# aoschu/esn-ofdm-mimo

Measured on AMD Instinct MI355X. Metric: OFDM symbols/s through the ESN detector (4x8 TDL-B, N=128, N_res=512; train+predict+detect), higher is better.
Workload: dtype f16 operands / f32 accumulate

## Files before the change

### esn_ofdm_mimo_amd/csrc/esn_solve.hip

```cpp
#include <stdlib.h>
#include "esn_common.h"

namespace esn {

struct SolveParams {
    const double* E; const double* D;
    const float* E32;
    int n_groups, T, transient, cols, n_out;
    const double* t_scale; const double* t_shift;
    double* W_out; int* status;
    double* work; size_t work_stride;
    int m, n, wide;
    int skip;
    int part_ok;
};

__device__ __forceinline__ double wave_sum(double v) {
#pragma unroll
    for (int off = 32; off > 0; off >>= 1) v += __shfl_down(v, off);
    return __shfl(v, 0);
}

__global__ __launch_bounds__(1024) void readout_qr_kernel(SolveParams sp) {
    __shared__ double red[16];
    __shared__ double bc[4];
    const int g = blockIdx.x;
    const int tid = threadIdx.x, nth = blockDim.x;
    const int lane = tid & 63, wv = tid >> 6, nwv = nth >> 6;
    const int m = sp.m, n = sp.n, nrhs = sp.n_out;
    const int rows = sp.T - sp.transient, cols = sp.cols;
    double* M = sp.work + (size_t)g * sp.work_stride;
    const int ncol_tot = sp.wide ? n : n + nrhs;
    double* R = M + (size_t)ncol_tot * m;
    double* rdiag = R + (size_t)nrhs * m;
    double* beta = rdiag + n;
    const double* Eg = sp.E + ((size_t)g * sp.T + sp.transient) * cols;
    const double* Dg = sp.D + ((size_t)g * sp.T + sp.transient) * nrhs;

    if (sp.wide) {
        for (size_t i = tid; i < (size_t)n * m; i += nth) M[i] = Eg[i];
        for (int i = tid; i < nrhs * m; i += nth) {
            int o = i / m, j = i % m;
            double v = 0.0;
            if (j < n) {
                double sc = sp.t_scale ? sp.t_scale[(size_t)g * nrhs + o] : 1.0;
                double sh = sp.t_shift ? sp.t_shift[(size_t)g * nrhs + o] : 0.0;
                v = Dg[(size_t)j * nrhs + o] * sc + sh;
            }
            R[i] = v;
        }
    } else {
        for (size_t i = tid; i < (size_t)n * m; i += nth) {
            int c = (int)(i / m), rr = (int)(i % m);
            M[i] = Eg[(size_t)rr * cols + c];
        }
        for (int i = tid; i < nrhs * m; i += nth) {
            int o = i / m, rr = i % m;
            double sc = sp.t_scale ? sp.t_scale[(size_t)g * nrhs + o] : 1.0;
            double sh = sp.t_shift ? sp.t_shift[(size_t)g * nrhs + o] : 0.0;
            M[(size_t)(n + o) * m + rr] = Dg[(size_t)rr * nrhs + o] * sc + sh;
        }
    }
    __syncthreads();

    for (int j = 0; j < n; ++j) {
        double* cj = M + (size_t)j * m;
        double part = 0.0;
        for (int i = j + tid; i < m; i += nth) { double x = cj[i]; part = fma(x, x, part); }
        part = wave_sum(part);
        if (lane == 0) red[wv] = part;
        __syncthreads();
        if (tid == 0) {
            double sigma = 0.0;
            for (int w = 0; w < nwv; ++w) sigma += red[w];
            double x0 = cj[j];
            double nx = sqrt(sigma);
            double alpha = (x0 >= 0.0) ? -nx : nx;
            double v0 = x0 - alpha;
            double vtv = sigma - x0 * x0 + v0 * v0;
            double b = (vtv > 0.0) ? 2.0 / vtv : 0.0;
            cj[j] = v0;
            rdiag[j] = alpha;
            beta[j] = b;
            bc[0] = b;
        }
        __syncthreads();
        const double b = bc[0];
        if (b != 0.0) {
            for (int c = j + 1 + wv; c < ncol_tot; c += nwv) {
                double* cc = M + (size_t)c * m;
                double dot = 0.0;
                for (int i = j + lane; i < m; i += 64) dot = fma(cj[i], cc[i], dot);
                dot = wave_sum(dot) * b;
                for (int i = j + lane; i < m; i += 64) cc[i] = fma(-dot, cj[i], cc[i]);
            }
        }
        __syncthreads();
    }

    double rmax = 0.0;
    for (int j = tid; j < n; j += nth) rmax = fmax(rmax, fabs(rdiag[j]));
#pragma unroll
    for (int off = 32; off > 0; off >>= 1) rmax = fmax(rmax, __shfl_down(rmax, off));
    if (lane == 0) red[wv] = rmax;
    __syncthreads();
    if (tid == 0) {
        double r = 0.0;
        for (int w = 0; w < nwv; ++w) r = fmax(r, red[w]);
        bc[1] = r * 1e-13;
        int bad = 0;
        for (int j = 0; j < n; ++j) bad |= (fabs(rdiag[j]) <= r * 1e-13);
        sp.status[g] = bad ? 1 : 0;
    }
    __syncthreads();
    const double tol = bc[1];

    if (sp.wide) {
        for (int o = wv; o < nrhs; o += nwv) {
            double* z = R + (size_t)o * m;
            for (int j = 0; j < n; ++j) {
                const double* cj = M + (size_t)j * m;
                double acc = 0.0;
                for (int k = lane; k < j; k += 64) acc = fma(cj[k], z[k], acc);
                acc = wave_sum(acc);
                if (lane == 0) {
                    double d = rdiag[j];
                    z[j] = (fabs(d) > tol) ? (z[j] - acc) / d : 0.0;
                }
                __builtin_amdgcn_s_waitcnt(0);
                __builtin_amdgcn_wave_barrier();
            }
            for (int j = n - 1; j >= 0; --j) {
                const double* cj = M + (size_t)j * m;
                const double b = beta[j];
                if (b == 0.0) continue;
                double dot = 0.0;
                for (int i = j + lane; i < m; i += 64) dot = fma(cj[i], z[i], dot);
                dot = wave_sum(dot) * b;
                for (int i = j + lane; i < m; i += 64) z[i] = fma(-dot, cj[i], z[i]);
                __builtin_amdgcn_s_waitcnt(0);
                __builtin_amdgcn_wave_barrier();
            }
            double* wo = sp.W_out + ((size_t)g * nrhs + o) * cols;
            for (int i = lane; i < m; i += 64) wo[i] = z[i];
        }
    } else {
        for (int o = wv; o < nrhs; o += nwv) {
            double* c = M + (size_t)(n + o) * m;
            for (int j = n - 1; j >= 0; --j) {
                double acc = 0.0;
                for (int k = j + 1 + lane; k < n; k += 64) acc = fma(M[(size_t)k * m + j], c[k], acc);
                acc = wave_sum(acc);
                if (lane == 0) {
                    double d = rdiag[j];
                    c[j] = (fabs(d) > tol) ? (c[j] - acc) / d : 0.0;
                }
                __builtin_amdgcn_s_waitcnt(0);
                __builtin_amdgcn_wave_barrier();
            }
            double* wo = sp.W_out + ((size_t)g * nrhs + o) * cols;
            for (int i = lane; i < n; i += 64) wo[i] = c[i];
        }
    }
}

size_t solve_work_doubles(int rows, int cols, int n_out) {
    const bool wide = rows < cols;
    const size_t m = wide ? cols : rows, n = wide ? rows : cols;
    size_t d = (n + (wide ? 0 : n_out)) * m + (size_t)n_out * m + 2 * n;
    return (d + 1) & ~(size_t)1;
}

int launch_readout_solve(const double* E, const double* D, int n_groups, int T, int transient,
                         int cols, int n_out, const double* t_scale, const double* t_shift,
                         double* W_out, int* status, void* workspace, hipStream_t stream) {
    SolveParams sp;
    const int rows = T - transient;
    sp.E = E; sp.E32 = nullptr; sp.D = D; sp.n_groups = n_groups; sp.T = T; sp.transient = transient;
    sp.cols = cols; sp.n_out = n_out; sp.t_scale = t_scale; sp.t_shift = t_shift;
    sp.W_out = W_out; sp.status = status;
    sp.work = reinterpret_cast<double*>(workspace);
    sp.work_stride = solve_work_doubles(rows, cols, n_out);
    sp.wide = rows < cols;
    sp.m = sp.wide ? cols : rows;
    sp.n = sp.wide ? rows : cols;
    hipLaunchKernelGGL(readout_qr_kernel, dim3(n_groups), dim3(1024), 0, stream, sp);
    return (int)hipGetLastError();
}

}

namespace esn {

constexpr int CH_NP = 128;
constexpr int CH_LD = CH_NP + 1;
constexpr int CH_KC = 32;

__global__ __launch_bounds__(1024) void readout_chol_kernel(SolveParams sp) {
    extern __shared__ __attribute__((aligned(16))) char chol_smem[];
    double* Gs = reinterpret_cast<double*>(chol_smem);
    double* As = Gs;
    double* Bs = Gs + CH_NP * CH_LD;
    __shared__ int sh_bad;
    const int g = blockIdx.x, tid = threadIdx.x;
    const int lane = tid & 63, wv = tid >> 6;
    const int rows = sp.T - sp.transient, cols = sp.cols, nrhs = sp.n_out;
    const bool wide = rows < cols;
    const int n = wide ? rows : cols;
    const int m = wide ? cols : rows;
    const size_t a_off = ((size_t)g * sp.T + sp.transient) * cols;
    const double* A = sp.E ? sp.E + a_off : nullptr;
    const float* A32 = sp.E32 ? sp.E32 + a_off : nullptr;
    const double* Dg = sp.D + ((size_t)g * sp.T + sp.transient) * nrhs;
    constexpr int AS_LD = CH_NP + 4;

    const int wvu = __builtin_amdgcn_readfirstlane(wv);
    const int g_cnt = (wvu >> 2) == 0 ? 3 : 2;
    int g_ti[3], g_tj[3];
#pragma unroll
    for (int q = 0; q < 3; ++q) {
        const int m = wvu >> 2;
        const int idx = m == 0 ? q : 2 * m + 1 + (q < 2 ? q : 0);
        const int t = 4 * idx + (wvu & 3);
        int ti = 0;
        while ((ti + 1) * (ti + 2) / 2 <= t) ++ti;
        g_ti[q] = ti;
        g_tj[q] = t - ti * (ti + 1) / 2;
    }
    typedef double f64x4 __attribute__((ext_vector_type(4)));
    f64x4 acc[3];
#pragma unroll
    for (int q = 0; q < 3; ++q) acc[q] = f64x4{0.0, 0.0, 0.0, 0.0};
    const int fr_off = (lane >> 4) * (CH_NP + 4) + (lane & 15);
    double atb = 0.0;
    const int ao = tid / CH_NP, ai = tid % CH_NP;
    constexpr int EPT = CH_KC * CH_NP / 1024;
    double stgA[EPT], stgB[EPT];
    auto fetch = [&](double (&stg)[EPT], int k0) {
#pragma unroll
        for (int q = 0; q < EPT; ++q) {
            const int e = tid + 1024 * q;
            int kk, i;
            if (wide) { i = e / CH_KC; kk = e % CH_KC; } else { kk = e / CH_NP; i = e % CH_NP; }
            const int k = k0 + kk;
            const size_t ai_ = wide ? (size_t)i * cols + k : (size_t)k * cols + i;
            stg[q] = (i < n && k < m) ? (A32 ? (double)A32[ai_] : A[ai_]) : 0.0;
        }
    };
    auto commit = [&](const double (&stg)[EPT], double* dst) {
#pragma unroll
        for (int q = 0; q < EPT; ++q) {
            const int e = tid + 1024 * q;
            int kk, i;
            if (wide) { i = e / CH_KC; kk = e % CH_KC; } else { kk = e / CH_NP; i = e % CH_NP; }
            dst[kk * AS_LD + i] = stg[q];
        }
    };
    double* Abuf[2] = {As, As + CH_KC * AS_LD};
    const int m_run = (sp.skip & 1) ? CH_KC : m;
    auto chunk = [&](int k0, int cur, const double (&stg_next)[EPT], double (&stg_free)[EPT]) {
        if (k0 + 2 * CH_KC < m_run) fetch(stg_free, k0 + 2 * CH_KC);
        const double* Ac = Abuf[cur];
        const int kmax = (m - k0 < CH_KC) ? m - k0 : CH_KC;
#pragma unroll 2
        for (int k4 = 0; k4 < CH_KC; k4 += 4) {
            const double* slab = Ac + k4 * AS_LD + fr_off;
#pragma unroll
            for (int q = 0; q < 3; ++q)
                if (q < g_cnt)
                    acc[q] = __builtin_amdgcn_mfma_f64_16x16x4f64(slab[g_ti[q] * 16], slab[g_tj[q] * 16], acc[q], 0, 0, 0);
        }
        if (!wide && ao < nrhs) {
            const double sc = sp.t_scale ? sp.t_scale[(size_t)g * nrhs + ao] : 1.0;
            const double sh = sp.t_shift ? sp.t_shift[(size_t)g * nrhs + ao] : 0.0;
            for (int kk = 0; kk < kmax; ++kk)
                atb = fma(Ac[kk * AS_LD + ai], Dg[(size_t)(k0 + kk) * nrhs + ao] * sc + sh, atb);
        }
        if (k0 + CH_KC < m_run) commit(stg_next, Abuf[cur ^ 1]);
        __syncthreads();
    };
    fetch(stgA, 0);
    commit(stgA, Abuf[0]);
    if (CH_KC < m_run) fetch(stgA, CH_KC);
    __syncthreads();
    for (int k0 = 0; k0 < m_run; k0 += 2 * CH_KC) {
        chunk(k0, 0, stgA, stgB);
        if (k0 + CH_KC < m_run) chunk(k0 + CH_KC, 1, stgB, stgA);
    }
    __syncthreads();
#pragma unroll
    for (int q = 0; q < 3; ++q)
        if (q < g_cnt) {
#pragma unroll
            for (int i = 0; i < 4; ++i)
                Gs[(g_ti[q] * 16 + 4 * i + (lane >> 4)) * CH_LD + g_tj[q] * 16 + (lane & 15)] = acc[q][i];
        }
    if (tid == 0) sh_bad = 0;
    for (int e = tid; e < nrhs * CH_NP; e += 1024) {
        const int o = e / CH_NP, i = e % CH_NP;
        double v = 0.0;
        if (wide && i < n) {
            const double sc = sp.t_scale ? sp.t_scale[(size_t)g * nrhs + o] : 1.0;
            const double sh = sp.t_shift ? sp.t_shift[(size_t)g * nrhs + o] : 0.0;
            v = Dg[(size_t)i * nrhs + o] * sc + sh;
        }
        if (wide) Bs[e] = v;
    }
    __syncthreads();
    if (!wide && ao < nrhs) Bs[ao * CH_NP + ai] = (ai < n) ? atb : 0.0;
    double dmax = 0.0;
    if (tid < n) dmax = Gs[tid * CH_LD + tid];
#pragma unroll
    for (int off = 32; off > 0; off >>= 1) dmax = fmax(dmax, __shfl_down(dmax, off));
    __shared__ double sh_max[2];
    if (tid < 128 && lane == 0) sh_max[wv] = dmax;
    __syncthreads();
    const double piv_tol = fmax(sh_max[0], sh_max[1]) * 1e-14;

    __shared__ double sh_invd[CH_NP];
    __shared__ double sh_linv[16][17];
    auto bcast = [](double x, int src) -> double {
        const uint64_t u = __builtin_bit_cast(uint64_t, x);
        const uint32_t lo = __builtin_amdgcn_readlane((uint32_t)u, src);
        const uint32_t hi = __builtin_amdgcn_readlane((uint32_t)(u >> 32), src);
        return __builtin_bit_cast(double, ((uint64_t)hi << 32) | lo);
    };
    const int nblk = (sp.skip & 2) ? 1 : (n + 15) / 16;
    const int lr = lane & 15, lq = lane >> 4;
    for (int kb = 0; kb < nblk; ++kb) {
        const int j0 = 16 * kb;
        if (wv == 0) {
            const int r = lane & 15;
            double a[16], x[16];
#pragma unroll
            for (int c = 0; c < 16; ++c) a[c] = Gs[(j0 + r) * CH_LD + j0 + c];
            double my_invd = 1.0;
            unsigned rejected = 0;
#pragma unroll
            for (int j = 0; j < 16; ++j) {
                const double v = bcast(a[j], j);
                const bool live = j0 + j < n;
                const bool ok = live && v > piv_tol;
                if (live && !ok) rejected |= 1u << j;
                const double d = ok ? sqrt(v) : 1.0, inv_d = ok ? 1.0 / d : 0.0;
                if (r == j) my_invd = ok ? inv_d : 1.0;
                a[j] = (r == j) ? d : ((r > j) ? a[j] * inv_d : 0.0);
#pragma unroll
                for (int k = j + 1; k < 16; ++k) {
                    const double lkj = bcast(a[j], k);
                    if (r >= k) a[k] = fma(-a[j], lkj, a[k]);
                }
            }
            if (lane < 16) {
#pragma unroll
                for (int c = 0; c < 16; ++c) Gs[(j0 + r) * CH_LD + j0 + c] = a[c];
                sh_invd[j0 + r] = my_invd;
            }
            if (rejected && lane == 0) sh_bad = 1;
#pragma unroll
            for (int i = 0; i < 16; ++i) {
                double sacc = (i == r) ? 1.0 : 0.0;
#pragma unroll
                for (int k = 0; k < i; ++k) sacc = fma(-bcast(a[k], i), x[k], sacc);
                const double idi = bcast(my_invd, i);
                x[i] = (i >= r && !((rejected >> i) & 1u)) ? sacc * idi : 0.0;
            }
            if (lane < 16) {
#pragma unroll
                for (int i = 0; i < 16; ++i) sh_linv[i][r] = x[i];
            }
        }
        __syncthreads();
        const int ntile = (n + 15) / 16;
        {
            const int rt = kb + 1 + wv;
            if (rt < ntile) {
                f64x4 c = {0.0, 0.0, 0.0, 0.0};
#pragma unroll
                for (int k0 = 0; k0 < 16; k0 += 4)
                    c = __builtin_amdgcn_mfma_f64_16x16x4f64(Gs[(rt * 16 + lr) * CH_LD + j0 + k0 + lq],
                                                             sh_linv[lr][k0 + lq], c, 0, 0, 0);
#pragma unroll
                for (int i = 0; i < 4; ++i) Gs[(rt * 16 + 4 * i + lq) * CH_LD + j0 + lr] = c[i];
            }
        }
        __syncthreads();
        {
            const int mt = ntile - kb - 1, cnt = mt * (mt + 1) / 2;
            for (int t = wv; t < cnt; t += 16) {
                int di = 0;
                while ((di + 1) * (di + 2) / 2 <= t) ++di;
                const int ti = kb + 1 + di, tj = kb + 1 + t - di * (di + 1) / 2;
                f64x4 c;
#pragma unroll
                for (int i = 0; i < 4; ++i) c[i] = Gs[(ti * 16 + 4 * i + lq) * CH_LD + tj * 16 + lr];
#pragma unroll
                for (int k0 = 0; k0 < 16; k0 += 4)
                    c = __builtin_amdgcn_mfma_f64_16x16x4f64(-Gs[(ti * 16 + lr) * CH_LD + j0 + k0 + lq],
                                                             Gs[(tj * 16 + lr) * CH_LD + j0 + k0 + lq], c, 0, 0, 0);
#pragma unroll
                for (int i = 0; i < 4; ++i) Gs[(ti * 16 + 4 * i + lq) * CH_LD + tj * 16 + lr] = c[i];
            }
        }
        __syncthreads();
    }

    for (int o = wv; o < ((sp.skip & 4) ? 0 : nrhs); o += 16) {
        double* x = Bs + o * CH_NP;
        double b0 = x[lane], b1 = x[lane + 64];
        for (int j = 0; j < n; ++j) {
            const double own = (j < 64) ? b0 : b1;
            const double zj = __shfl(own, j & 63) * sh_invd[j];
            if (lane == (j & 63)) { if (j < 64) b0 = zj; else b1 = zj; }
            const double l0 = (lane > j) ? Gs[lane * CH_LD + j] : 0.0;
            const double l1 = (lane + 64 > j && lane + 64 < n) ? Gs[(lane + 64) * CH_LD + j] : 0.0;
            b0 = fma(-l0, zj, b0);
            b1 = fma(-l1, zj, b1);
        }
        for (int j = n - 1; j >= 0; --j) {
            const double own = (j < 64) ? b0 : b1;
            const double xj = __shfl(own, j & 63) * sh_invd[j];
            if (lane == (j & 63)) { if (j < 64) b0 = xj; else b1 = xj; }
            const double* Lj = Gs + j * CH_LD;
            const double l0 = (lane < j) ? Lj[lane] : 0.0;
            const double l1 = (lane + 64 < j) ? Lj[lane + 64] : 0.0;
            b0 = fma(-l0, xj, b0);
            b1 = fma(-l1, xj, b1);
        }
        x[lane] = b0; x[lane + 64] = b1;
    }
    __syncthreads();

    if (wide) {
        const int npair = cols / 2;
        if ((cols & 1) == 0 && 3 * npair <= 1024 && 3 * npair * 16 <= CH_NP * CH_LD && !(sp.skip & 8)) {
            double* part = Gs;
            const int third = tid / npair, pr = tid - third * npair;
            if (third < 3) {
                const int per = (n + 2) / 3;
                const int i0 = third * per, i1 = (i0 + per < n) ? i0 + per : n;
                double w0[8], w1[8];
#pragma unroll
                for (int o = 0; o < 8; ++o) { w0[o] = 0.0; w1[o] = 0.0; }
                const size_t ac = 2 * (size_t)pr;
#pragma unroll 8
                for (int i = i0; i < i1; ++i) {
                    double2 a;
                    if (A32) {
                        const float2 af = *reinterpret_cast<const float2*>(A32 + ac + (size_t)i * cols);
                        a = double2{(double)af.x, (double)af.y};
                    } else {
                        a = *reinterpret_cast<const double2*>(A + ac + (size_t)i * cols);
                    }
#pragma unroll
                    for (int o = 0; o < 8; ++o)
                        if (o < nrhs) {
                            const double al = Bs[o * CH_NP + i];
                            w0[o] = fma(a.x, al, w0[o]);
                            w1[o] = fma(a.y, al, w1[o]);
                        }
                }
#pragma unroll
                for (int o = 0; o < 8; ++o)
                    if (o < nrhs) {
                        part[(third * 8 + o) * cols + 2 * pr] = w0[o];
                        part[(third * 8 + o) * cols + 2 * pr + 1] = w1[o];
                    }
            }
            __syncthreads();
            for (int e = tid; e < nrhs * cols; e += 1024) {
                const int o = e / cols, c = e - o * cols;
                sp.W_out[((size_t)g * nrhs + o) * cols + c] =
                    (part[o * cols + c] + part[(8 + o) * cols + c]) + part[(16 + o) * cols + c];
            }
        } else {
            for (int c = tid; c < ((sp.skip & 8) ? 0 : cols); c += 1024) {
                double w[8];
#pragma unroll
                for (int o = 0; o < 8; ++o) w[o] = 0.0;
#pragma unroll 8
                for (int i = 0; i < n; ++i) {
                    const double a = A32 ? (double)A32[(size_t)i * cols + c] : A[(size_t)i * cols + c];
#pragma unroll
                    for (int o = 0; o < 8; ++o)
                        if (o < nrhs) w[o] = fma(a, Bs[o * CH_NP + i], w[o]);
                }
#pragma unroll
                for (int o = 0; o < 8; ++o)
                    if (o < nrhs) sp.W_out[((size_t)g * nrhs + o) * cols + c] = w[o];
            }
        }
    } else {
        for (int e = tid; e < nrhs * cols; e += 1024) {
            const int o = e / cols, c = e % cols;
            sp.W_out[((size_t)g * nrhs + o) * cols + c] = Bs[o * CH_NP + c];
        }
    }
    if (tid == 0) sp.status[g] = sh_bad;
}

int launch_readout_chol(const double* E, const float* E32, const double* D, int n_groups, int T, int transient,
                        int cols, int n_out, const double* t_scale, const double* t_shift,
                        double* W_out, int* status, hipStream_t stream) {
    SolveParams sp;
    sp.E32 = E32;
    const int rows = T - transient;
    const int n = rows < cols ? rows : cols;
    if (n > CH_NP || n_out > 8) return -1;
    sp.E = E; sp.D = D; sp.n_groups = n_groups; sp.T = T; sp.transient = transient;
    sp.cols = cols; sp.n_out = n_out; sp.t_scale = t_scale; sp.t_shift = t_shift;
    sp.W_out = W_out; sp.status = status; sp.work = nullptr; sp.work_stride = 0;
    sp.wide = rows < cols; sp.m = sp.wide ? cols : rows; sp.n = n;
    sp.skip = knobs().chol_skip;
    const size_t lds = sizeof(double) * ((size_t)CH_NP * CH_LD + (size_t)n_out * CH_NP);
    hipError_t e = hipFuncSetAttribute(reinterpret_cast<const void*>(readout_chol_kernel),
                                       hipFuncAttributeMaxDynamicSharedMemorySize, (int)lds);
    if (e != hipSuccess) return (int)e;
    hipLaunchKernelGGL(readout_chol_kernel, dim3(n_groups), dim3(1024), lds, stream, sp);
    return (int)hipGetLastError();
}

}

namespace esn {

constexpr int CB_NMAX = 512;
constexpr int CB_KC = 8;
constexpr int CB_PLD = 17;
constexpr int CB_NT = 512;
constexpr int CB_NW = CB_NT / 64;
constexpr int CB_EPT = CB_NMAX * CB_KC / CB_NT;
constexpr int CB_TPW = 16;

size_t chol_big_work_doubles(int n) {
    const size_t np = (size_t)round_up(n, 16);
    return np * np;
}

__global__ __launch_bounds__(CB_NT) void readout_chol_big_kernel(SolveParams sp) {
    extern __shared__ __attribute__((aligned(16))) char cb_smem[];
    typedef double f64x4 __attribute__((ext_vector_type(4)));
    __shared__ int sh_bad;
    __shared__ double sh_invd[CB_NMAX];
    __shared__ double sh_linv[16][17];
    __shared__ double sh_red[CB_NW];
    const int g = blockIdx.x, tid = threadIdx.x;
    const int lane = tid & 63, wv = tid >> 6;
    const int wvu = __builtin_amdgcn_readfirstlane(wv);
    const int rows = sp.T - sp.transient, cols = sp.cols, nrhs = sp.n_out;
    const bool wide = rows < cols;
    const int n = wide ? rows : cols;
    const int m = wide ? cols : rows;
    const int np = round_up(n, 16), ntile = np / 16;
    const int ld = np;
    double* Gw = sp.work + (size_t)g * sp.work_stride;
    const size_t a_off = ((size_t)g * sp.T + sp.transient) * cols;
    const double* A = sp.E ? sp.E + a_off : nullptr;
    const float* A32 = sp.E32 ? sp.E32 + a_off : nullptr;
    const double* Dg = sp.D + ((size_t)g * sp.T + sp.transient) * nrhs;
    const int lr = lane & 15, lq = lane >> 4;
    if (tid == 0) sh_bad = 0;

    {
        const int AS_LD = np + 4;
        double* Abuf[2] = {reinterpret_cast<double*>(cb_smem), reinterpret_cast<double*>(cb_smem) + (size_t)CB_KC * AS_LD};
        const int ept = (np * CB_KC + CB_NT - 1) / CB_NT;
        double stg[CB_EPT];
        auto fetch = [&](int k0) {
#pragma unroll
            for (int q = 0; q < CB_EPT; ++q) {
                const int e = tid + CB_NT * q;
                int kk, i;
                if (wide) { i = e / CB_KC; kk = e % CB_KC; } else { kk = e / np; i = e % np; }
                const int k = k0 + kk;
                const size_t ai_ = wide ? (size_t)i * cols + k : (size_t)k * cols + i;
                stg[q] = (q < ept && e < np * CB_KC && i < n && k < m) ? (A32 ? (double)A32[ai_] : A[ai_]) : 0.0;
            }
        };
        auto commit = [&](double* dst) {
#pragma unroll
            for (int q = 0; q < CB_EPT; ++q) {
                const int e = tid + CB_NT * q;
                if (q < ept && e < np * CB_KC) {
                    int kk, i;
                    if (wide) { i = e / CB_KC; kk = e % CB_KC; } else { kk = e / np; i = e % np; }
                    dst[kk * AS_LD + i] = stg[q];
                }
            }
        };
        const int fr_off = lq * AS_LD + lr;
        const int n_pass = (ntile + 3) / 4;
        for (int jb = 0; jb < n_pass; ++jb) {
            const int tj0 = 4 * jb, tj1 = (tj0 + 4 < ntile) ? tj0 + 4 : ntile;
            int cnt = 0;
            for (int tj = tj0; tj < tj1; ++tj) cnt += ntile - tj;
            int my_ti[CB_TPW], my_tj[CB_TPW];
#pragma unroll
            for (int q = 0; q < CB_TPW; ++q) {
                int t = wvu + CB_NW * q, tj = tj0;
                bool ok = t < cnt;
                while (ok && t >= ntile - tj) { t -= ntile - tj; ++tj; }
                my_tj[q] = ok ? tj : -1;
                my_ti[q] = ok ? tj + t : 0;
            }
            f64x4 acc[CB_TPW];
#pragma unroll
            for (int q = 0; q < CB_TPW; ++q) acc[q] = f64x4{0.0, 0.0, 0.0, 0.0};
            fetch(0);
            commit(Abuf[0]);
            __syncthreads();
            int cur = 0;
            for (int k0 = 0; k0 < m; k0 += CB_KC) {
                const bool more = k0 + CB_KC < m;
                if (more) fetch(k0 + CB_KC);
                const double* Ac = Abuf[cur];
#pragma unroll
                for (int k4 = 0; k4 < CB_KC; k4 += 4) {
                    const double* slab = Ac + k4 * AS_LD + fr_off;
#pragma unroll
                    for (int q = 0; q < CB_TPW; ++q)
                        if (my_tj[q] >= 0)
                            acc[q] = __builtin_amdgcn_mfma_f64_16x16x4f64(slab[my_ti[q] * 16], slab[my_tj[q] * 16], acc[q], 0, 0, 0);
                }
                if (more) commit(Abuf[cur ^ 1]);
                __syncthreads();
                cur ^= 1;
            }
#pragma unroll
            for (int q = 0; q < CB_TPW; ++q)
                if (my_tj[q] >= 0) {
#pragma unroll
                    for (int i = 0; i < 4; ++i)
                        Gw[(size_t)(my_tj[q] * 16 + lr) * ld + my_ti[q] * 16 + 4 * i + lq] = acc[q][i];
                }
            __syncthreads();
        }
        double* Bs = reinterpret_cast<double*>(cb_smem);
        __syncthreads();
        for (int e = tid; e < nrhs * np; e += CB_NT) {
            const int o = e / np, i = e % np;
            double v = 0.0;
            if (wide && i < n) {
                const double sc = sp.t_scale ? sp.t_scale[(size_t)g * nrhs + o] : 1.0;
                const double sh = sp.t_shift ? sp.t_shift[(size_t)g * nrhs + o] : 0.0;
                v = Dg[(size_t)i * nrhs + o] * sc + sh;
            }
            if (wide) Bs[e] = v;
        }
        if (!wide) {
            for (int e = tid; e < nrhs * np; e += CB_NT) {
                const int o = e / np, i = e % np;
                double acc_b = 0.0;
                if (i < n) {
                    const double sc = sp.t_scale ? sp.t_scale[(size_t)g * nrhs + o] : 1.0;
                    const double sh = sp.t_shift ? sp.t_shift[(size_t)g * nrhs + o] : 0.0;
#pragma unroll 8
                    for (int k = 0; k < m; ++k) {
                        const double a = A32 ? (double)A32[(size_t)k * cols + i] : A[(size_t)k * cols + i];
                        acc_b = fma(a, Dg[(size_t)k * nrhs + o] * sc + sh, acc_b);
                    }
                }
                Bs[e] = acc_b;
            }
        }
    }
    __threadfence_block();
    __syncthreads();
    double* Bs = reinterpret_cast<double*>(cb_smem);
    double* P = Bs + (size_t)8 * CB_NMAX;
    double dmax = 0.0;
    for (int i = tid; i < n; i += CB_NT) dmax = fmax(dmax, Gw[(size_t)i * ld + i]);
#pragma unroll
    for (int off = 32; off > 0; off >>= 1) dmax = fmax(dmax, __shfl_down(dmax, off));
    if (lane == 0) sh_red[wv] = dmax;
    __syncthreads();
    double piv_tol = 0.0;
    for (int w = 0; w < CB_NW; ++w) piv_tol = fmax(piv_tol, sh_red[w]);
    piv_tol *= 1e-14;

    auto bcast = [](double x, int src) -> double {
        const uint64_t u = __builtin_bit_cast(uint64_t, x);
        const uint32_t lo = __builtin_amdgcn_readlane((uint32_t)u, src);
        const uint32_t hi = __builtin_amdgcn_readlane((uint32_t)(u >> 32), src);
        return __builtin_bit_cast(double, ((uint64_t)hi << 32) | lo);
    };
    for (int j = 0; j < ntile; ++j) {
        const int j0 = 16 * j;
        for (int rt = j + wvu; rt < ntile; rt += CB_NW) {
            f64x4 c;
#pragma unroll
            for (int i = 0; i < 4; ++i) c[i] = Gw[(size_t)(j0 + lr) * ld + rt * 16 + 4 * i + lq];
            const double* la = Gw + (size_t)lq * ld + rt * 16 + lr;
            const double* lb = Gw + (size_t)lq * ld + j0 + lr;
#pragma unroll 4
            for (int k = 0; k < j0; k += 4)
                c = __builtin_amdgcn_mfma_f64_16x16x4f64(-la[(size_t)k * ld], lb[(size_t)k * ld], c, 0, 0, 0);
#pragma unroll
            for (int i = 0; i < 4; ++i) P[(rt * 16 + 4 * i + lq) * CB_PLD + lr] = c[i];
        }
        __syncthreads();
        if (wv == 0) {
            const int r = lane & 15;
            double a[16], x[16];
#pragma unroll
            for (int c = 0; c < 16; ++c) a[c] = P[(j0 + r) * CB_PLD + c];
            double my_invd = 1.0;
            unsigned rejected = 0;
#pragma unroll
            for (int jj = 0; jj < 16; ++jj) {
                const double v = bcast(a[jj], jj);
                const bool live = j0 + jj < n;
                const bool ok = live && v > piv_tol;
                if (live && !ok) rejected |= 1u << jj;
                const double d = ok ? sqrt(v) : 1.0, inv_d = ok ? 1.0 / d : 0.0;
                if (r == jj) my_invd = ok ? inv_d : 1.0;
                a[jj] = (r == jj) ? d : ((r > jj) ? a[jj] * inv_d : 0.0);
#pragma unroll
                for (int k = jj + 1; k < 16; ++k) {
                    const double lkj = bcast(a[jj], k);
                    if (r >= k) a[k] = fma(-a[jj], lkj, a[k]);
                }
            }
            if (lane < 16) {
#pragma unroll
                for (int c = 0; c < 16; ++c) P[(j0 + r) * CB_PLD + c] = a[c];
                sh_invd[j0 + r] = my_invd;
            }
            if (rejected && lane == 0) sh_bad = 1;
#pragma unroll
            for (int i = 0; i < 16; ++i) {
                double sacc = (i == r) ? 1.0 : 0.0;
#pragma unroll
                for (int k = 0; k < i; ++k) sacc = fma(-bcast(a[k], i), x[k], sacc);
                const double idi = bcast(my_invd, i);
                x[i] = (i >= r && !((rejected >> i) & 1u)) ? sacc * idi : 0.0;
            }
            if (lane < 16) {
#pragma unroll
                for (int i = 0; i < 16; ++i) sh_linv[i][r] = x[i];
            }
        }
        __syncthreads();
        for (int rt = j + 1 + wvu; rt < ntile; rt += CB_NW) {
            f64x4 c = {0.0, 0.0, 0.0, 0.0};
#pragma unroll
            for (int k0 = 0; k0 < 16; k0 += 4)
                c = __builtin_amdgcn_mfma_f64_16x16x4f64(P[(rt * 16 + lr) * CB_PLD + k0 + lq], sh_linv[lr][k0 + lq], c, 0, 0, 0);
            __builtin_amdgcn_wave_barrier();
#pragma unroll
            for (int i = 0; i < 4; ++i) P[(rt * 16 + 4 * i + lq) * CB_PLD + lr] = c[i];
        }
        __syncthreads();
        for (int e = tid; e < (np - j0) * 16; e += CB_NT) {
            const int c = e / (np - j0), rr = j0 + e % (np - j0);
            Gw[(size_t)(j0 + c) * ld + rr] = P[rr * CB_PLD + c];
        }
        __threadfence_block();
        __syncthreads();
    }

    if (wv < nrhs) {
        double* xb = Bs + (size_t)wv * np;
        constexpr int NS = CB_NMAX / 64;
        const int ns = (np + 63) / 64;
        double b[NS], l[NS], lnext[NS];
#pragma unroll
        for (int s2 = 0; s2 < NS; ++s2) b[s2] = (s2 < ns && lane + 64 * s2 < np) ? xb[lane + 64 * s2] : 0.0;
        auto load_col = [&](double (&dst)[NS], int jc) {
#pragma unroll
            for (int s2 = 0; s2 < NS; ++s2) {
                const int i = lane + 64 * s2;
                dst[s2] = (s2 < ns && jc >= 0 && jc < n && i < n) ? Gw[(size_t)jc * ld + i] : 0.0;
            }
        };
        auto pick = [&](const double (&v)[NS], int jc) -> double {
            double own = 0.0;
#pragma unroll
            for (int s2 = 0; s2 < NS; ++s2) own = ((jc >> 6) == s2) ? v[s2] : own;
            return __shfl(own, jc & 63);
        };
        load_col(l, 0);
        for (int jc = 0; jc < n; ++jc) {
            load_col(lnext, jc + 1);
            const double zj = pick(b, jc) * sh_invd[jc];
#pragma unroll
            for (int s2 = 0; s2 < NS; ++s2) {
                const int i = lane + 64 * s2;
                b[s2] = (i == jc) ? zj : ((i > jc) ? fma(-l[s2], zj, b[s2]) : b[s2]);
            }
#pragma unroll
            for (int s2 = 0; s2 < NS; ++s2) l[s2] = lnext[s2];
        }
        load_col(l, n - 1);
        for (int jc = n - 1; jc >= 0; --jc) {
            load_col(lnext, jc - 1);
            double part = 0.0;
#pragma unroll
            for (int s2 = 0; s2 < NS; ++s2) {
                const int i = lane + 64 * s2;
                part = (i > jc && i < n) ? fma(l[s2], b[s2], part) : part;
            }
            part = wave_sum(part);
            const double xj = (pick(b, jc) - part) * sh_invd[jc];
#pragma unroll
            for (int s2 = 0; s2 < NS; ++s2) b[s2] = (lane + 64 * s2 == jc) ? xj : b[s2];
#pragma unroll
            for (int s2 = 0; s2 < NS; ++s2) l[s2] = lnext[s2];
        }
#pragma unroll
        for (int s2 = 0; s2 < NS; ++s2)
            if (s2 < ns && lane + 64 * s2 < np) xb[lane + 64 * s2] = b[s2];
    }
    __syncthreads();

    if (wide) {
        double* part = P;
        if (sp.part_ok) {
            const int cpt = A32 ? 4 : 2, nunit = cols / cpt;
            int parts = CB_NT / nunit;
            if (parts > 3) parts = 3;
            const int pt = tid / nunit, un = tid - pt * nunit;
// ... 108 lines not shown
```

Baseline: 10.25 million.

## Restructure Cholesky readout kernel with packed tile storage and 512-thread blocks

Rewrites the small-n Cholesky readout solve to keep the Gram matrix as packed lower-triangular 16x16 tiles with an XOR swizzle, instead of a padded dense array. The block size drops from 1024 to 512 threads with a waves-per-EU hint so more blocks can be resident. The kernel is templated on element type and on wide/tall shape, and gains vectorised float4/double2 loads of E plus a column-vectorised W_out back-projection. The triangular solves use MFMA on the tiles, and fewer LDS bytes per block are meant to raise occupancy. In exchange each wave handles more tiles and the solve phases carry more synchronisation and complexity.

Result: faster. 10.88 million, median of 6 (+6.1%).

```diff
diff --git a/esn_ofdm_mimo_amd/csrc/esn_solve.hip b/esn_ofdm_mimo_amd/csrc/esn_solve.hip
--- a/esn_ofdm_mimo_amd/csrc/esn_solve.hip
+++ b/esn_ofdm_mimo_amd/csrc/esn_solve.hip
@@ -13,6 +13,7 @@
     int m, n, wide;
     int skip;
     int part_ok;
+    int vec;
 };
 
 __device__ __forceinline__ double wave_sum(double v) {
@@ -193,310 +194,407 @@
 namespace esn {
 
 constexpr int CH_NP = 128;
-constexpr int CH_LD = CH_NP + 1;
+constexpr int CH_NT = 512;
+constexpr int CH_NW = CH_NT / 64;
+constexpr int CH_TILES = 36;
 constexpr int CH_KC = 32;
-
-__global__ __launch_bounds__(1024) void readout_chol_kernel(SolveParams sp) {
+constexpr int CH_AS_LD = CH_NP + 16;
+constexpr int CH_RHS = 8;
+constexpr size_t CH_LDS = sizeof(double) * ((size_t)CH_TILES * 256 + (size_t)CH_NP * CH_RHS);
+static_assert(2 * CH_KC * CH_AS_LD <= CH_TILES * 256, "E staging aliases the Gram tiles");
+
+typedef double f64x4 __attribute__((ext_vector_type(4)));
+
+__device__ __forceinline__ int ch_tile(int ti, int tj) { return (ti * (ti + 1) / 2 + tj) * 256; }
+__device__ __forceinline__ int ch_el(int r, int c) { return r * 16 + (c ^ (r & ~1)); }
+
+__device__ __forceinline__ void ch_load4(const float* p, float (&v)[4]) {
+    const float4 x = *reinterpret_cast<const float4*>(p);
+    v[0] = x.x; v[1] = x.y; v[2] = x.z; v[3] = x.w;
+}
+__device__ __forceinline__ void ch_load4(const double* p, double (&v)[4]) {
+    const double2 x = *reinterpret_cast<const double2*>(p), y = *reinterpret_cast<const double2*>(p + 2);
+    v[0] = x.x; v[1] = x.y; v[2] = y.x; v[3] = y.y;
+}
+__device__ __forceinline__ const float* ch_src(const SolveParams& sp, float*) { return sp.E32; }
+__device__ __forceinline__ const double* ch_src(const SolveParams& sp, double*) { return sp.E; }
+
+__device__ __forceinline__ double ch_bcast(double x, int src) {
+    const uint64_t u = __builtin_bit_cast(uint64_t, x);
+    const uint32_t lo = __builtin_amdgcn_readlane((uint32_t)u, src);
+    const uint32_t hi = __builtin_amdgcn_readlane((uint32_t)(u >> 32), src);
+    return __builtin_bit_cast(double, ((uint64_t)hi << 32) | lo);
+}
+
+__device__ __forceinline__ int ch_factor_diag(double* D, int j0, int n, double piv_tol, int lane) {
+    const int r = lane & 15;
+    double a[16], x[16];
+#pragma unroll
+    for (int c = 0; c < 16; ++c) a[c] = D[ch_el(r, c)];
+    double my_invd = 1.0;
+    unsigned rejected = 0, dropped = 0;
+#pragma unroll
+    for (int j = 0; j < 16; ++j) {
+        const double v = ch_bcast(a[j], j);
+        const bool live = j0 + j < n;
+        const bool ok = live && v > piv_tol;
+        if (live && !ok) rejected |= 1u << j;
+        if (!ok) dropped |= 1u << j;
+        const double d = ok ? sqrt(v) : 1.0, inv_d = ok ? 1.0 / d : 0.0;
+        if (r == j) my_invd = ok ? inv_d : 1.0;
+        a[j] = (r == j) ? d : ((r > j) ? a[j] * inv_d : 0.0);
+#pragma unroll
+        for (int k = j + 1; k < 16; ++k) {
+            const double lkj = ch_bcast(a[j], k);
+            if (r >= k) a[k] = fma(-a[j], lkj, a[k]);
+        }
+    }
+#pragma unroll
+    for (int i = 0; i < 16; ++i) {
+        double sacc = (i == r) ? 1.0 : 0.0;
+#pragma unroll
+        for (int k = 0; k < i; ++k) sacc = fma(-ch_bcast(a[k], i), x[k], sacc);
+        const double idi = ch_bcast(my_invd, i);
+        x[i] = (i >= r && !((dropped >> i) & 1u)) ? sacc * idi : 0.0;
+    }
+    if (lane < 16) {
+#pragma unroll
+        for (int i = 0; i < 16; ++i) D[ch_el(i, r)] = x[i];
+    }
+    return rejected ? 1 : 0;
+}
+
+template <typename TE, bool wide>
+__global__ __launch_bounds__(CH_NT) __attribute__((amdgpu_waves_per_eu(4))) void readout_chol_kernel(SolveParams sp) {
     extern __shared__ __attribute__((aligned(16))) char chol_smem[];
     double* Gs = reinterpret_cast<double*>(chol_smem);
     double* As = Gs;
-    double* Bs = Gs + CH_NP * CH_LD;
-    __shared__ int sh_bad;
+    double* Bs = Gs + CH_TILES * 256;
     const int g = blockIdx.x, tid = threadIdx.x;
-    const int lane = tid & 63, wv = tid >> 6;
+    const int lane = tid & 63, wv = __builtin_amdgcn_readfirstlane(tid >> 6);
+    const int lr = lane & 15, lq = lane >> 4;
     const int rows = sp.T - sp.transient, cols = sp.cols, nrhs = sp.n_out;
-    const bool wide = rows < cols;
     const int n = wide ? rows : cols;
     const int m = wide ? cols : rows;
-    const size_t a_off = ((size_t)g * sp.T + sp.transient) * cols;
-    const double* A = sp.E ? sp.E + a_off : nullptr;
-    const float* A32 = sp.E32 ? sp.E32 + a_off : nullptr;
+    const int ntile = (n + 15) / 16;
+    const TE* A = ch_src(sp, (TE*)nullptr) + ((size_t)g * sp.T + sp.transient) * cols;
     const double* Dg = sp.D + ((size_t)g * sp.T + sp.transient) * nrhs;
-    constexpr int AS_LD = CH_NP + 4;
-
-    const int wvu = __builtin_amdgcn_readfirstlane(wv);
-    const int g_cnt = (wvu >> 2) == 0 ? 3 : 2;
-    int g_ti[3], g_tj[3];
-#pragma unroll
-    for (int q = 0; q < 3; ++q) {
-        const int m = wvu >> 2;
-        const int idx = m == 0 ? q : 2 * m + 1 + (q < 2 ? q : 0);
-        const int t = 4 * idx + (wvu & 3);
+
+    int g_ti[5], g_tj[5];
+    const int g_cnt = wv < 4 ? 5 : 4;
+#pragma unroll
+    for (int q = 0; q < 5; ++q) {
+        const int t = wv + CH_NW * q < CH_TILES ? wv + CH_NW * q : 0;
         int ti = 0;
         while ((ti + 1) * (ti + 2) / 2 <= t) ++ti;
         g_ti[q] = ti;
         g_tj[q] = t - ti * (ti + 1) / 2;
     }
-    typedef double f64x4 __attribute__((ext_vector_type(4)));
-    f64x4 acc[3];
-#pragma unroll
-    for (int q = 0; q < 3; ++q) acc[q] = f64x4{0.0, 0.0, 0.0, 0.0};
-    const int fr_off = (lane >> 4) * (CH_NP + 4) + (lane & 15);
-    double atb = 0.0;
-    const int ao = tid / CH_NP, ai = tid % CH_NP;
-    constexpr int EPT = CH_KC * CH_NP / 1024;
-    double stgA[EPT], stgB[EPT];
-    auto fetch = [&](double (&stg)[EPT], int k0) {
-#pragma unroll
-        for (int q = 0; q < EPT; ++q) {
-            const int e = tid + 1024 * q;
-            int kk, i;
-            if (wide) { i = e / CH_KC; kk = e % CH_KC; } else { kk = e / CH_NP; i = e % CH_NP; }
+    f64x4 acc[5];
+#pragma unroll
+    for (int q = 0; q < 5; ++q) acc[q] = f64x4{0.0, 0.0, 0.0, 0.0};
+    double atb[2] = {0.0, 0.0};
+    auto run_of = [&](int p, int& i, int& kk) {
+        const int e = tid + CH_NT * p;
+        if (wide) { i = (e & 15) + 16 * ((e >> 7) & 7); kk = 4 * ((e >> 4) & 7); }
+        else      { kk = e >> 5; i = 4 * (e & 31); }
+    };
+    TE stg[2][4];
+    auto fetch = [&](int k0) {
+#pragma unroll
+        for (int p = 0; p < 2; ++p) {
+            int i, kk;
+            run_of(p, i, kk);
             const int k = k0 + kk;
-            const size_t ai_ = wide ? (size_t)i * cols + k : (size_t)k * cols + i;
-            stg[q] = (i < n && k < m) ? (A32 ? (double)A32[ai_] : A[ai_]) : 0.0;
+            int nv = wide ? (i < n ? m - k : 0) : (k < m ? n - i : 0);
+            nv = nv < 0 ? 0 : (nv > 4 ? 4 : nv);
+            const TE* src = A + (wide ? (size_t)i * cols + k : (size_t)k * cols + i);
+            if (nv == 4 && sp.vec) {
+                ch_load4(src, stg[p]);
+            } else {
+#pragma unroll
+                for (int j = 0; j < 4; ++j) stg[p][j] = j < nv ? src[j] : (TE)0;
+            }
         }
     };
-    auto commit = [&](const double (&stg)[EPT], double* dst) {
-#pragma unroll
-        for (int q = 0; q < EPT; ++q) {
-            const int e = tid + 1024 * q;
-            int kk, i;
-            if (wide) { i = e / CH_KC; kk = e % CH_KC; } else { kk = e / CH_NP; i = e % CH_NP; }
-            dst[kk * AS_LD + i] = stg[q];
+    auto commit = [&](double* dst) {
+#pragma unroll
+        for (int p = 0; p < 2; ++p) {
+            int i, kk;
+            run_of(p, i, kk);
+#pragma unroll
+            for (int j = 0; j < 4; ++j) {
+                if (wide) dst[(kk + j) * CH_AS_LD + i] = (double)stg[p][j];
+                else      dst[kk * CH_AS_LD + i + j] = (double)stg[p][j];
+            }
         }
     };
-    double* Abuf[2] = {As, As + CH_KC * AS_LD};
+    double* Abuf[2] = {As, As + CH_KC * CH_AS_LD};
     const int m_run = (sp.skip & 1) ? CH_KC : m;
-    auto chunk = [&](int k0, int cur, const double (&stg_next)[EPT], double (&stg_free)[EPT]) {
-        if (k0 + 2 * CH_KC < m_run) fetch(stg_free, k0 + 2 * CH_KC);
+    for (int k0 = 0, cur = 0; k0 < m_run; k0 += CH_KC, cur ^= 1) {
+        if (k0 == 0) {
+            fetch(0);
+            commit(Abuf[0]);
+            __syncthreads();
+        }
+        if (k0 + CH_KC < m_run) fetch(k0 + CH_KC);
         const double* Ac = Abuf[cur];
         const int kmax = (m - k0 < CH_KC) ? m - k0 : CH_KC;
-#pragma unroll 2
-        for (int k4 = 0; k4 < CH_KC; k4 += 4) {
-            const double* slab = Ac + k4 * AS_LD + fr_off;
-#pragma unroll
-            for (int q = 0; q < 3; ++q)
+        const double* slab0 = Ac + lq * CH_AS_LD + lr;
+        for (int k4 = 0; k4 < kmax; k4 += 4) {
+            const double* slab = slab0 + k4 * CH_AS_LD;
+#pragma unroll
+            for (int q = 0; q < 5; ++q)
                 if (q < g_cnt)
                     acc[q] = __builtin_amdgcn_mfma_f64_16x16x4f64(slab[g_ti[q] * 16], slab[g_tj[q] * 16], acc[q], 0, 0, 0);
         }
-        if (!wide && ao < nrhs) {
-            const double sc = sp.t_scale ? sp.t_scale[(size_t)g * nrhs + ao] : 1.0;
-            const double sh = sp.t_shift ? sp.t_shift[(size_t)g * nrhs + ao] : 0.0;
-            for (int kk = 0; kk < kmax; ++kk)
-                atb = fma(Ac[kk * AS_LD + ai], Dg[(size_t)(k0 + kk) * nrhs + ao] * sc + sh, atb);
-        }
-        if (k0 + CH_KC < m_run) commit(stg_next, Abuf[cur ^ 1]);
-        __syncthreads();
-    };
-    fetch(stgA, 0);
-    commit(stgA, Abuf[0]);
-    if (CH_KC < m_run) fetch(stgA, CH_KC);
+        if constexpr (!wide) {
+#pragma unroll
+            for (int p = 0; p < 2; ++p) {
+                const int e = tid + CH_NT * p, o = e / CH_NP, i = e % CH_NP;
+                if (o < nrhs) {
+                    const double sc = sp.t_scale ? sp.t_scale[(size_t)g * nrhs + o] : 1.0;
+                    const double sh = sp.t_shift ? sp.t_shift[(size_t)g * nrhs + o] : 0.0;
+                    for (int kk = 0; kk < kmax; ++kk)
+                        atb[p] = fma(Ac[kk * CH_AS_LD + i], Dg[(size_t)(k0 + kk) * nrhs + o] * sc + sh, atb[p]);
+                }
+            }
+        }
+        if (k0 + CH_KC < m_run) commit(Abuf[cur ^ 1]);
+        __syncthreads();
+    }
+
+#pragma unroll
+    for (int q = 0; q < 5; ++q)
+        if (q < g_cnt) {
+            double* T = Gs + ch_tile(g_ti[q], g_tj[q]);
+#pragma unroll
+            for (int i = 0; i < 4; ++i) T[ch_el(4 * i + lq, lr)] = acc[q][i];
+        }
+#pragma unroll
+    for (int p = 0; p < 2; ++p) {
+        const int e = tid + CH_NT * p;
+        if (wide) {
+            const int i = e / CH_RHS, o = e % CH_RHS;
+            double v = 0.0;
+            if (i < n && o < nrhs) {
+                const double sc = sp.t_scale ? sp.t_scale[(size_t)g * nrhs + o] : 1.0;
+                const double sh = sp.t_shift ? sp.t_shift[(size_t)g * nrhs + o] : 0.0;
+                v = Dg[(size_t)i * nrhs + o] * sc + sh;
+            }
+            Bs[e] = v;
+        } else {
+            const int o = e / CH_NP, i = e % CH_NP;
+            Bs[i * CH_RHS + o] = (o < nrhs && i < n) ? atb[p] : 0.0;
+        }
+    }
     __syncthreads();
-    for (int k0 = 0; k0 < m_run; k0 += 2 * CH_KC) {
-        chunk(k0, 0, stgA, stgB);
-        if (k0 + CH_KC < m_run) chunk(k0 + CH_KC, 1, stgB, stgA);
-    }
-    __syncthreads();
-#pragma unroll
-    for (int q = 0; q < 3; ++q)
-        if (q < g_cnt) {
-#pragma unroll
-            for (int i = 0; i < 4; ++i)
-                Gs[(g_ti[q] * 16 + 4 * i + (lane >> 4)) * CH_LD + g_tj[q] * 16 + (lane & 15)] = acc[q][i];
-        }
-    if (tid == 0) sh_bad = 0;
-    for (int e = tid; e < nrhs * CH_NP; e += 1024) {
-        const int o = e / CH_NP, i = e % CH_NP;
-        double v = 0.0;
-        if (wide && i < n) {
-            const double sc = sp.t_scale ? sp.t_scale[(size_t)g * nrhs + o] : 1.0;
-            const double sh = sp.t_shift ? sp.t_shift[(size_t)g * nrhs + o] : 0.0;
-            v = Dg[(size_t)i * nrhs + o] * sc + sh;
-        }
-        if (wide) Bs[e] = v;
-    }
-    __syncthreads();
-    if (!wide && ao < nrhs) Bs[ao * CH_NP + ai] = (ai < n) ? atb : 0.0;
-    double dmax = 0.0;
-    if (tid < n) dmax = Gs[tid * CH_LD + tid];
-#pragma unroll
-    for (int off = 32; off > 0; off >>= 1) dmax = fmax(dmax, __shfl_down(dmax, off));
-    __shared__ double sh_max[2];
-    if (tid < 128 && lane == 0) sh_max[wv] = dmax;
-    __syncthreads();
-    const double piv_tol = fmax(sh_max[0], sh_max[1]) * 1e-14;
-
-    __shared__ double sh_invd[CH_NP];
-    __shared__ double sh_linv[16][17];
-    auto bcast = [](double x, int src) -> double {
-        const uint64_t u = __builtin_bit_cast(uint64_t, x);
-        const uint32_t lo = __builtin_amdgcn_readlane((uint32_t)u, src);
-        const uint32_t hi = __builtin_amdgcn_readlane((uint32_t)(u >> 32), src);
-        return __builtin_bit_cast(double, ((uint64_t)hi << 32) | lo);
-    };
-    const int nblk = (sp.skip & 2) ? 1 : (n + 15) / 16;
-    const int lr = lane & 15, lq = lane >> 4;
-    for (int kb = 0; kb < nblk; ++kb) {
-        const int j0 = 16 * kb;
-        if (wv == 0) {
-            const int r = lane & 15;
-            double a[16], x[16];
-#pragma unroll
-            for (int c = 0; c < 16; ++c) a[c] = Gs[(j0 + r) * CH_LD + j0 + c];
-            double my_invd = 1.0;
-            unsigned rejected = 0;
-#pragma unroll
-            for (int j = 0; j < 16; ++j) {
-                const double v = bcast(a[j], j);
-                const bool live = j0 + j < n;
-                const bool ok = live && v > piv_tol;
-                if (live && !ok) rejected |= 1u << j;
-                const double d = ok ? sqrt(v) : 1.0, inv_d = ok ? 1.0 / d : 0.0;
-                if (r == j) my_invd = ok ? inv_d : 1.0;
-                a[j] = (r == j) ? d : ((r > j) ? a[j] * inv_d : 0.0);
-#pragma unroll
-                for (int k = j + 1; k < 16; ++k) {
-                    const double lkj = bcast(a[j], k);
-                    if (r >= k) a[k] = fma(-a[j], lkj, a[k]);
-                }
-            }
-            if (lane < 16) {
-#pragma unroll
-                for (int c = 0; c < 16; ++c) Gs[(j0 + r) * CH_LD + j0 + c] = a[c];
-                sh_invd[j0 + r] = my_invd;
-            }
-            if (rejected && lane == 0) sh_bad = 1;
-#pragma unroll
-            for (int i = 0; i < 16; ++i) {
-                double sacc = (i == r) ? 1.0 : 0.0;
-#pragma unroll
-                for (int k = 0; k < i; ++k) sacc = fma(-bcast(a[k], i), x[k], sacc);
-                const double idi = bcast(my_invd, i);
-                x[i] = (i >= r && !((rejected >> i) & 1u)) ? sacc * idi : 0.0;
-            }
-            if (lane < 16) {
-#pragma unroll
-                for (int i = 0; i < 16; ++i) sh_linv[i][r] = x[i];
-            }
-        }
-        __syncthreads();
-        const int ntile = (n + 15) / 16;
-        {
+
+    int bad = 0;
+    const int nblk = (sp.skip & 2) ? 1 : ntile;
+    double piv_tol = 0.0;
+    if (wv == 0) {
+        double dmax = 0.0;
+        for (int i = lane; i < n; i += 64) dmax = fmax(dmax, Gs[ch_tile(i >> 4, i >> 4) + ch_el(i & 15, i & 15)]);
+#pragma unroll
+        for (int off = 32; off > 0; off >>= 1) dmax = fmax(dmax, __shfl_xor(dmax, off));
+        piv_tol = dmax * 1e-14;
+    }
+    for (int kb = -1; kb < nblk; ++kb) {
+        if (kb >= 0) {
             const int rt = kb + 1 + wv;
             if (rt < ntile) {
+                const double* Li = Gs + ch_tile(kb, kb);
+
+                double* T = Gs + ch_tile(rt, kb);
                 f64x4 c = {0.0, 0.0, 0.0, 0.0};
 #pragma unroll
                 for (int k0 = 0; k0 < 16; k0 += 4)
-                    c = __builtin_amdgcn_mfma_f64_16x16x4f64(Gs[(rt * 16 + lr) * CH_LD + j0 + k0 + lq],
-                                                             sh_linv[lr][k0 + lq], c, 0, 0, 0);
-#pragma unroll
-                for (int i = 0; i < 4; ++i) Gs[(rt * 16 + 4 * i + lq) * CH_LD + j0 + lr] = c[i];
-            }
-        }
-        __syncthreads();
-        {
+                    c = __builtin_amdgcn_mfma_f64_16x16x4f64(T[ch_el(lr, k0 + lq)], Li[ch_el(lr, k0 + lq)], c, 0, 0, 0);
+#pragma unroll
+                for (int i = 0; i < 4; ++i) T[ch_el(4 * i + lq, lr)] = c[i];
+            }
+        }
+        if (kb >= 0) {
+            __syncthreads();
             const int mt = ntile - kb - 1, cnt = mt * (mt + 1) / 2;
-            for (int t = wv; t < cnt; t += 16) {
+            for (int t = wv; t < cnt; t += (wv == 0 ? cnt : CH_NW - 1)) {
                 int di = 0;
                 while ((di + 1) * (di + 2) / 2 <= t) ++di;
                 const int ti = kb + 1 + di, tj = kb + 1 + t - di * (di + 1) / 2;
+                double* C = Gs + ch_tile(ti, tj);
+                const double* La = Gs + ch_tile(ti, kb);
+                const double* Lb = Gs + ch_tile(tj, kb);
                 f64x4 c;
 #pragma unroll
-                for (int i = 0; i < 4; ++i) c[i] = Gs[(ti * 16 + 4 * i + lq) * CH_LD + tj * 16 + lr];
+                for (int i = 0; i < 4; ++i) c[i] = C[ch_el(4 * i + lq, lr)];
 #pragma unroll
                 for (int k0 = 0; k0 < 16; k0 += 4)
-                    c = __builtin_amdgcn_mfma_f64_16x16x4f64(-Gs[(ti * 16 + lr) * CH_LD + j0 + k0 + lq],
-                                                             Gs[(tj * 16 + lr) * CH_LD + j0 + k0 + lq], c, 0, 0, 0);
-#pragma unroll
-                for (int i = 0; i < 4; ++i) Gs[(ti * 16 + 4 * i + lq) * CH_LD + tj * 16 + lr] = c[i];
-            }
-        }
-        __syncthreads();
-    }
-
-    for (int o = wv; o < ((sp.skip & 4) ? 0 : nrhs); o += 16) {
-        double* x = Bs + o * CH_NP;
-        double b0 = x[lane], b1 = x[lane + 64];
-        for (int j = 0; j < n; ++j) {
-            const double own = (j < 64) ? b0 : b1;
-            const double zj = __shfl(own, j & 63) * sh_invd[j];
-            if (lane == (j & 63)) { if (j < 64) b0 = zj; else b1 = zj; }
-            const double l0 = (lane > j) ? Gs[lane * CH_LD + j] : 0.0;
-            const double l1 = (lane + 64 > j && lane + 64 < n) ? Gs[(lane + 64) * CH_LD + j] : 0.0;
-            b0 = fma(-l0, zj, b0);
-            b1 = fma(-l1, zj, b1);
-        }
-        for (int j = n - 1; j >= 0; --j) {
-            const double own = (j < 64) ? b0 : b1;
-            const double xj = __shfl(own, j & 63) * sh_invd[j];
-            if (lane == (j & 63)) { if (j < 64) b0 = xj; else b1 = xj; }
-            const double* Lj = Gs + j * CH_LD;
-            const double l0 = (lane < j) ? Lj[lane] : 0.0;
-            const double l1 = (lane + 64 < j) ? Lj[lane + 64] : 0.0;
-            b0 = fma(-l0, xj, b0);
-            b1 = fma(-l1, xj, b1);
-        }
-        x[lane] = b0; x[lane + 64] = b1;
-    }
-    __syncthreads();
-
-    if (wide) {
-        const int npair = cols / 2;
-        if ((cols & 1) == 0 && 3 * npair <= 1024 && 3 * npair * 16 <= CH_NP * CH_LD && !(sp.skip & 8)) {
+                    c = __builtin_amdgcn_mfma_f64_16x16x4f64(-La[ch_el(lr, k0 + lq)], Lb[ch_el(lr, k0 + lq)], c, 0, 0, 0);
+#pragma unroll
+                for (int i = 0; i < 4; ++i) C[ch_el(4 * i + lq, lr)] = c[i];
+            }
+        }
+        if (wv == 0 && kb + 1 < nblk) bad |= ch_factor_diag(Gs + ch_tile(kb + 1, kb + 1), 16 * (kb + 1), n, piv_tol, lane);
+        __syncthreads();
+    }
+
+    if (!(sp.skip & 4)) {
+        const bool bl = lr < CH_RHS;
+        f64x4 keep = {0.0, 0.0, 0.0, 0.0};
+        int keep_t = -1;
+        auto rhs_tile = [&](int I) -> f64x4 {
+            f64x4 v;
+#pragma unroll
+            for (int i = 0; i < 4; ++i) v[i] = bl ? Bs[(16 * I + 4 * i + lq) * CH_RHS + lr] : 0.0;
+            return v;
+        };
+        auto put_tile = [&](int I, const f64x4& v) {
+            if (bl) {
+#pragma unroll
+                for (int i = 0; i < 4; ++i) Bs[(16 * I + 4 * i + lq) * CH_RHS + lr] = v[i];
+            }
+        };
+        auto flush = [&]() {
+            if (wv == CH_NW - 1 && keep_t >= 0) put_tile(keep_t, keep);
+            keep_t = -1;
+        };
+        for (int I = 0; I < ntile; ++I) {
+            flush();
+            const int J = I + 1 + wv;
+            const bool upd = J < ntile;
+            if (upd || wv == CH_NW - 1) {
+                const double* Li = Gs + ch_tile(I, I);
+                const f64x4 b = rhs_tile(I);
+                f64x4 z = {0.0, 0.0, 0.0, 0.0};
+#pragma unroll
+                for (int s = 0; s < 4; ++s)
+                    z = __builtin_amdgcn_mfma_f64_16x16x4f64(Li[ch_el(lr, 4 * s + lq)], b[s], z, 0, 0, 0);
+                if (upd) {
+                    const double* L = Gs + ch_tile(J, I);
+                    f64x4 c = rhs_tile(J);
+#pragma unroll
+                    for (int s = 0; s < 4; ++s)
+                        c = __builtin_amdgcn_mfma_f64_16x16x4f64(-L[ch_el(lr, 4 * s + lq)], z[s], c, 0, 0, 0);
+                    put_tile(J, c);
+                } else {
+                    keep = z;
+                    keep_t = I;
+                }
+            }
+            __syncthreads();
+        }
+        flush();
+        __syncthreads();
+        for (int I = ntile - 1; I >= 0; --I) {
+            flush();
+            const int J = wv;
+            const bool upd = J < I;
+            if (upd || wv == CH_NW - 1) {
+                const double* Li = Gs + ch_tile(I, I);
+                const f64x4 zi = rhs_tile(I);
+                f64x4 x = {0.0, 0.0, 0.0, 0.0};
+#pragma unroll
+                for (int s = 0; s < 4; ++s)
+                    x = __builtin_amdgcn_mfma_f64_16x16x4f64(Li[ch_el(4 * s + lq, lr)], zi[s], x, 0, 0, 0);
+                if (upd) {
+                    const double* L = Gs + ch_tile(I, J);
+                    f64x4 c = rhs_tile(J);
+#pragma unroll
+                    for (int s = 0; s < 4; ++s)
+                        c = __builtin_amdgcn_mfma_f64_16x16x4f64(-L[ch_el(4 * s + lq, lr)], x[s], c, 0, 0, 0);
+                    put_tile(J, c);
+                } else {
+                    keep = x;
+                    keep_t = I;
+                }
+            }
+            __syncthreads();
+        }
+        flush();
+        __syncthreads();
+    }
+
+    if constexpr (wide) {
+        constexpr int CPT = 16 / sizeof(TE);
+        const int nunit = cols / CPT;
+        int parts = nunit > 0 ? CH_NT / nunit : 0;
+        parts = parts > 3 ? 3 : parts;
+        if (sp.vec && cols % CPT == 0 && parts > 0 && (parts - 1) * CH_RHS * cols <= CH_TILES * 256 && !(sp.skip & 8)) {
             double* part = Gs;
-            const int third = tid / npair, pr = tid - third * npair;
-            if (third < 3) {
-                const int per = (n + 2) / 3;
-                const int i0 = third * per, i1 = (i0 + per < n) ? i0 + per : n;
-                double w0[8], w1[8];
-#pragma unroll
-                for (int o = 0; o < 8; ++o) { w0[o] = 0.0; w1[o] = 0.0; }
-                const size_t ac = 2 * (size_t)pr;
-#pragma unroll 8
+            const int pt = tid / nunit, un = tid - pt * nunit;
+            double w[CPT][CH_RHS];
+#pragma unroll
+            for (int c = 0; c < CPT; ++c)
+#pragma unroll
+                for (int o = 0; o < CH_RHS; ++o) w[c][o] = 0.0;
+            if (pt < parts) {
+                const int per = (n + parts - 1) / parts;
+                const int i0 = pt * per, i1 = (i0 + per < n) ? i0 + per : n;
+                const TE* ac = A + (size_t)CPT * un;
+#pragma unroll 4
                 for (int i = i0; i < i1; ++i) {
-                    double2 a;
-                    if (A32) {
-                        const float2 af = *reinterpret_cast<const float2*>(A32 + ac + (size_t)i * cols);
-                        a = double2{(double)af.x, (double)af.y};
+                    TE a[CPT];
+                    if constexpr (CPT == 4) {
+                        ch_load4(ac + (size_t)i * cols, a);
                     } else {
-                        a = *reinterpret_cast<const double2*>(A + ac + (size_t)i * cols);
+                        const double2 ad = *reinterpret_cast<const double2*>(ac + (size_t)i * cols);
+                        a[0] = ad.x; a[1] = ad.y;
                     }
 #pragma unroll
-                    for (int o = 0; o < 8; ++o)
+                    for (int o = 0; o < CH_RHS; ++o)
                         if (o < nrhs) {
-                            const double al = Bs[o * CH_NP + i];
-                            w0[o] = fma(a.x, al, w0[o]);
-                            w1[o] = fma(a.y, al, w1[o]);
+                            const double al = Bs[i * CH_RHS + o];
+#pragma unroll
+                            for (int c = 0; c < CPT; ++c) w[c][o] = fma((double)a[c], al, w[c][o]);
                         }
                 }
-#pragma unroll
-                for (int o = 0; o < 8; ++o)
+                if (pt > 0) {
+#pragma unroll
+                    for (int o = 0; o < CH_RHS; ++o)
+                        if (o < nrhs) {
+#pragma unroll
+                            for (int c = 0; c < CPT; ++c) part[((pt - 1) * CH_RHS + o) * cols + CPT * un + c] = w[c][o];
+                        }
+                }
+            }
+            __syncthreads();
+            if (pt == 0) {
+#pragma unroll
+                for (int o = 0; o < CH_RHS; ++o)
                     if (o < nrhs) {
-                        part[(third * 8 + o) * cols + 2 * pr] = w0[o];
-                        part[(third * 8 + o) * cols + 2 * pr + 1] = w1[o];
+#pragma unroll
+                        for (int c = 0; c < CPT; ++c) {
+                            double v = w[c][o];
+                            for (int q = 1; q < parts; ++q) v += part[((q - 1) * CH_RHS + o) * cols + CPT * un + c];
+                            sp.W_out[((size_t)g * nrhs + o) * cols + CPT * un + c] = v;
+                        }
                     }
             }
-            __syncthreads();
-            for (int e = tid; e < nrhs * cols; e += 1024) {
-                const int o = e / cols, c = e - o * cols;
-                sp.W_out[((size_t)g * nrhs + o) * cols + c] =
-                    (part[o * cols + c] + part[(8 + o) * cols + c]) + part[(16 + o) * cols + c];
-            }
         } else {
-            for (int c = tid; c < ((sp.skip & 8) ? 0 : cols); c += 1024) {
-                double w[8];
-#pragma unroll
-                for (int o = 0; o < 8; ++o) w[o] = 0.0;
+            for (int c = tid; c < ((sp.skip & 8) ? 0 : cols); c += CH_NT) {
+                double w[CH_RHS];
+#pragma unroll
+                for (int o = 0; o < CH_RHS; ++o) w[o] = 0.0;
 #pragma unroll 8
                 for (int i = 0; i < n; ++i) {
-                    const double a = A32 ? (double)A32[(size_t)i * cols + c] : A[(size_t)i * cols + c];
-#pragma unroll
-                    for (int o = 0; o < 8; ++o)
-                        if (o < nrhs) w[o] = fma(a, Bs[o * CH_NP + i], w[o]);
-                }
-#pragma unroll
-                for (int o = 0; o < 8; ++o)
+                    const double a = (double)A[(size_t)i * cols + c];
+#pragma unroll
+                    for (int o = 0; o < CH_RHS; ++o)
+                        if (o < nrhs) w[o] = fma(a, Bs[i * CH_RHS + o], w[o]);
+                }
+#pragma unroll
+                for (int o = 0; o < CH_RHS; ++o)
                     if (o < nrhs) sp.W_out[((size_t)g * nrhs + o) * cols + c] = w[o];
             }
         }
     } else {
-        for (int e = tid; e < nrhs * cols; e += 1024) {
+        for (int e = tid; e < nrhs * cols; e += CH_NT) {
             const int o = e / cols, c = e % cols;
-            sp.W_out[((size_t)g * nrhs + o) * cols + c] = Bs[o * CH_NP + c];
-        }
-    }
-    if (tid == 0) sp.status[g] = sh_bad;
+            sp.W_out[((size_t)g * nrhs + o) * cols + c] = Bs[c * CH_RHS + o];
+        }
+    }
+    if (tid == 0) sp.status[g] = bad;
 }
 
 int launch_readout_chol(const double* E, const float* E32, const double* D, int n_groups, int T, int transient,
@@ -506,17 +604,21 @@
     sp.E32 = E32;
     const int rows = T - transient;
     const int n = rows < cols ? rows : cols;
-    if (n > CH_NP || n_out > 8) return -1;
+    if (n > CH_NP || n_out > CH_RHS) return -1;
     sp.E = E; sp.D = D; sp.n_groups = n_groups; sp.T = T; sp.transient = transient;
     sp.cols = cols; sp.n_out = n_out; sp.t_scale = t_scale; sp.t_shift = t_shift;
     sp.W_out = W_out; sp.status = status; sp.work = nullptr; sp.work_stride = 0;
     sp.wide = rows < cols; sp.m = sp.wide ? cols : rows; sp.n = n;
     sp.skip = knobs().chol_skip;
-    const size_t lds = sizeof(double) * ((size_t)CH_NP * CH_LD + (size_t)n_out * CH_NP);
-    hipError_t e = hipFuncSetAttribute(reinterpret_cast<const void*>(readout_chol_kernel),
-                                       hipFuncAttributeMaxDynamicSharedMemorySize, (int)lds);
+    sp.part_ok = 0;
+    const uintptr_t base = E32 ? (uintptr_t)E32 : (uintptr_t)E;
+    sp.vec = (base % 16 == 0) && (cols % (E32 ? 4 : 2) == 0);
+    void (*fn)(SolveParams) = E32 ? (sp.wide ? readout_chol_kernel<float, true> : readout_chol_kernel<float, false>)
+                                  : (sp.wide ? readout_chol_kernel<double, true> : readout_chol_kernel<double, false>);
+    hipError_t e = hipFuncSetAttribute(reinterpret_cast<const void*>(fn), hipFuncAttributeMaxDynamicSharedMemorySize,
+                                       (int)CH_LDS);
     if (e != hipSuccess) return (int)e;
-    hipLaunchKernelGGL(readout_chol_kernel, dim3(n_groups), dim3(1024), lds, stream, sp);
+    hipLaunchKernelGGL(fn, dim3(n_groups), dim3(CH_NT), CH_LDS, stream, sp);
     return (int)hipGetLastError();
 }
 
```
